# facebookresearch/esm

Measured on NVIDIA H100. Metric: sequences/sec ESM-2 650M L=1024 embedding extract, higher is better.
Workload: dtype f16 operands, f32 accumulate/residual/LayerNorm/softmax

## Files before the change

### esm_b200/csrc/api.cu

```cuda
#include "../../include/esmb200.h"

#include <cuda.h>
#include <cuda_runtime.h>
#include <stdio.h>
#include <stdlib.h>
#include <string.h>

#include <string>
#include <vector>

#include <mutex>

#include "attention8.cuh"
#include "attention_contact.cuh"
#include "attention_probs.cuh"
#include "common.cuh"
#include "elementwise.cuh"
#include "gemm2.cuh"
#include "gemm_fp8.cuh"
#include "jacobian.cuh"
#include "msa_select.cuh"
#include "sampling.cuh"
#include "tied_attention.cuh"

using namespace esmb200;

namespace {

thread_local std::string g_last_error;

int fail(int code, const std::string& msg) {
  g_last_error = msg;
  return code;
}

int fail_cuda(cudaError_t e, const char* what) {
  if (e == cudaErrorMemoryAllocation)
    return fail(ESMB200_ENOMEM, std::string("CUDA out of memory. (") + what + ")");
  return fail(ESMB200_ECUDA, std::string(what) + ": " + cudaGetErrorString(e));
}

#define CK(expr)                                        \
  do {                                                  \
    cudaError_t _e = (expr);                            \
    if (_e != cudaSuccess) return fail_cuda(_e, #expr); \
  } while (0)


enum ProfTag : int { T_LN1 = 0, T_QKV, T_ATTN, T_OUT, T_LN2, T_FC1, T_FC2, T_KEYBITS, T_EMBED, T_LN_F32, T_PROBS,
                     T_CONVERT, T_GEMM_OTHER, T_MEANPOOL, T_TIED_SCORES, T_TIED_SOFTMAX, T_TIED_PV, T_LOG_SOFTMAX,
                     T_WINDOW_MERGE, T_JACOBIAN, T_SAMPLING, T_MSA_SELECT, T_COUNT };
struct Profiler {
  std::mutex mu;
  bool on = false;
  std::vector<cudaEvent_t> ev;
  std::vector<int> tag;
  size_t used = 0;
  long long launches = 0;
};
Profiler g_prof;

struct ProfScope {
  cudaStream_t st;
  bool rec;
  size_t slot = 0;
  ProfScope(int tag, cudaStream_t s) : st(s), rec(false) {
    std::lock_guard<std::mutex> lk(g_prof.mu);
    ++g_prof.launches;
    if (g_prof.on && g_prof.used + 2 <= g_prof.ev.size()) {
      rec = true;
      slot = g_prof.used;
      g_prof.used += 2;
      g_prof.tag.push_back(tag);
      cudaEventRecord(g_prof.ev[slot], st);
    }
  }
  ~ProfScope() {
    if (rec) cudaEventRecord(g_prof.ev[slot + 1], st);
  }
};

typedef CUresult (*EncodeTiledFn)(CUtensorMap*, CUtensorMapDataType, cuuint32_t, void*, const cuuint64_t*,
                                  const cuuint64_t*, const cuuint32_t*, const cuuint32_t*, CUtensorMapInterleave,
                                  CUtensorMapSwizzle, CUtensorMapL2promotion, CUtensorMapFloatOOBfill);

EncodeTiledFn get_encode_fn() {
  static EncodeTiledFn fn = nullptr;
  if (fn) return fn;
  void* p = nullptr;
  cudaDriverEntryPointQueryResult qres;
  if (cudaGetDriverEntryPoint("cuTensorMapEncodeTiled", &p, cudaEnableDefault, &qres) != cudaSuccess ||
      qres != cudaDriverEntryPointSuccess)
    return nullptr;
  fn = reinterpret_cast<EncodeTiledFn>(p);
  return fn;
}

int make_tmap_2d(CUtensorMap* map, const void* ptr, int esize, uint64_t rows, uint64_t cols, uint64_t ld_elems,
                 uint32_t box_rows) {
  EncodeTiledFn enc = get_encode_fn();
  if (!enc) return fail(ESMB200_ECUDA, "cuTensorMapEncodeTiled entry point not available");
  if ((reinterpret_cast<uintptr_t>(ptr) & 15) != 0 || (ld_elems * esize) % 16 != 0)
    return fail(ESMB200_EINVAL, "TMA operand must be 16-byte aligned with a 16-byte multiple row pitch");
  cuuint64_t dims[2] = {cols, rows};
  cuuint64_t strides[1] = {ld_elems * (uint64_t)esize};
  cuuint32_t box[2] = {(cuuint32_t)(128 / esize), box_rows};
  cuuint32_t estr[2] = {1, 1};
  const CUtensorMapDataType dt = esize == 1   ? CU_TENSOR_MAP_DATA_TYPE_UINT8
                                 : esize == 2 ? CU_TENSOR_MAP_DATA_TYPE_FLOAT16
                                              : CU_TENSOR_MAP_DATA_TYPE_FLOAT32;
  CUresult r = enc(map, dt, 2,
                   const_cast<void*>(ptr), dims, strides, box, estr,
                   CU_TENSOR_MAP_INTERLEAVE_NONE, CU_TENSOR_MAP_SWIZZLE_128B, CU_TENSOR_MAP_L2_PROMOTION_L2_256B,
                   CU_TENSOR_MAP_FLOAT_OOB_FILL_NONE);
  if (r != CUDA_SUCCESS) {
    char buf[160];
    snprintf(buf, sizeof buf, "cuTensorMapEncodeTiled failed (%d) rows=%llu cols=%llu ld=%llu box_rows=%u", (int)r,
             (unsigned long long)rows, (unsigned long long)cols, (unsigned long long)ld_elems, box_rows);
    return fail(ESMB200_ECUDA, buf);
  }
  return ESMB200_OK;
}

int make_tmap_f16(CUtensorMap* map, const void* ptr, uint64_t rows, uint64_t cols, uint64_t ld_elems,
                  uint32_t box_rows) {
  return make_tmap_2d(map, ptr, 2, rows, cols, ld_elems, box_rows);
}

int make_gemm_out_map(CUtensorMap* map, const void* out, int esize, uint64_t rows, uint64_t cols) {
  return make_tmap_2d(map, out, esize, rows, cols, cols, gemm2_cfg::OUT_BOX_ROWS);
}

inline int head_slots(int E, int H) { return (H > 0 && E / H > 64) ? 2 : 1; }

constexpr int kMaxDevices = 64;

int num_sms() {
  static int n[kMaxDevices] = {};
  int dev = 0;
  cudaGetDevice(&dev);
  if (dev < 0 || dev >= kMaxDevices) dev = 0;
  if (n[dev] == 0) cudaDeviceGetAttribute(&n[dev], cudaDevAttrMultiProcessorCount, dev);
  return n[dev];
}

int check_device() {
  static int ok[kMaxDevices] = {};
  int dev = 0;
  if (cudaGetDevice(&dev) != cudaSuccess) return fail(ESMB200_ECUDA, "no CUDA device");
  if (dev < 0 || dev >= kMaxDevices) return fail(ESMB200_ECUDA, "device ordinal out of range");
  if (ok[dev] == 0) {
    int major = 0;
    cudaDeviceGetAttribute(&major, cudaDevAttrComputeCapabilityMajor, dev);
    ok[dev] = (major == 9) ? 1 : -1;
  }
  if (ok[dev] < 0)
    return fail(ESMB200_ECUDA, "esmb200 requires an sm_90a (Hopper H100) device; there is no fallback path");
  return ESMB200_OK;
}

size_t align_up(size_t v, size_t a) { return (v + a - 1) / a * a; }

constexpr int kContactMaxS = 1024;
const char* const kContactMaxSMsg = "contact head supports at most 1024 positions";

template <bool SPLIT>
cudaError_t launch_gemm_epi(int epi, const CUtensorMap& ta, const CUtensorMap& tb, const CUtensorMap& to,
                            const GemmParams& p, cudaStream_t st) {
  switch (epi) {
    case EPI_QKV_ROPE: return launch_gemm2_epi<EPI_QKV_ROPE, SPLIT>(ta, tb, to, p, num_sms(), st);
    case EPI_BIAS_RESIDUAL: return launch_gemm2_epi<EPI_BIAS_RESIDUAL, SPLIT>(ta, tb, to, p, num_sms(), st);
    case EPI_BIAS_GELU: return launch_gemm2_epi<EPI_BIAS_GELU, SPLIT>(ta, tb, to, p, num_sms(), st);
    case EPI_BIAS_F32: return launch_gemm2_epi<EPI_BIAS_F32, SPLIT>(ta, tb, to, p, num_sms(), st);
    case EPI_BIAS_GELU_F32: return launch_gemm2_epi<EPI_BIAS_GELU_F32, SPLIT>(ta, tb, to, p, num_sms(), st);
    default: return cudaErrorInvalidValue;
  }
}

int launch_gemm(int epi, const CUtensorMap& ta, const CUtensorMap& tb, const CUtensorMap& to, const GemmParams& p,
                cudaStream_t st, int tag = T_GEMM_OTHER, bool split = false) {
  ProfScope ps(tag, st);
  if (split && p.K % 64 != 0) return fail(ESMB200_EINVAL, "fp32x3 precision needs K % 64 == 0");
  if (epi < EPI_QKV_ROPE || epi > EPI_BIAS_GELU_F32) return fail(ESMB200_EINVAL, "unknown GEMM epilogue");
  const cudaError_t e =
      split ? launch_gemm_epi<true>(epi, ta, tb, to, p, st) : launch_gemm_epi<false>(epi, ta, tb, to, p, st);
  if (e != cudaSuccess) return fail_cuda(e, split ? "gemm launch (fp32x3)" : "gemm launch");
  return ESMB200_OK;
}

int launch_gemm_fp8(int epi, const CUtensorMap& ta, const CUtensorMap& tb, const CUtensorMap& to, const Fp8GemmParams& p,
                    cudaStream_t st, int tag = T_GEMM_OTHER) {
  ProfScope ps(tag, st);
  cudaError_t e;
  switch (epi) {
    case EPI_QKV_ROPE: e = launch_gemm_fp8_epi<EPI_QKV_ROPE>(ta, tb, to, p, num_sms(), st); break;
    case EPI_BIAS_RESIDUAL: e = launch_gemm_fp8_epi<EPI_BIAS_RESIDUAL>(ta, tb, to, p, num_sms(), st); break;
    case EPI_GELU_FP8: e = launch_gemm_fp8_epi<EPI_GELU_FP8>(ta, tb, to, p, num_sms(), st); break;
    default: return fail(ESMB200_EINVAL, "fp8 gemm epilogue must be 0 (qkv), 1 (residual) or 5 (gelu -> fp8)");
  }
  if (e != cudaSuccess) return fail_cuda(e, "gemm launch (fp8)");
  return ESMB200_OK;
}

inline int kblocks(int K) { return (K + 127) / 128; }

GemmParams gemm_params(int M, int N, int K, const float* bias) {
  GemmParams g;
  memset(&g, 0, sizeof g);
  g.M = M; g.N = N; g.K = K; g.bias = bias;
  return g;
}

struct AttnScratch {
  uint32_t* keybits;
  int* kvlen;
  float* row_max;
  float* row_sum;
  int words;
  size_t bytes;
};

AttnScratch attn_scratch_layout(uintptr_t base, int B, int T, int H) {
  AttnScratch s;
  s.words = (int)align_up((size_t)(T + 31) / 32, 4);
  const size_t keybits = align_up((size_t)B * s.words * 4, 256), kvlen = align_up((size_t)B * 4, 256);
  const size_t stats = align_up((size_t)B * H * T * 4, 256);
  s.keybits = reinterpret_cast<uint32_t*>(base);
  s.kvlen = reinterpret_cast<int*>(base + keybits);
  s.row_max = reinterpret_cast<float*>(base + keybits + kvlen);
  s.row_sum = reinterpret_cast<float*>(base + keybits + kvlen + stats);
  s.bytes = keybits + kvlen + 2 * stats;
  return s;
}

int run_key_bits(const uint8_t* pad_mask, const AttnScratch& s, int B, int T, cudaStream_t st) {
  const int wpb = 4;
  ProfScope ps(T_KEYBITS, st);
  key_bits_kernel<<<(B + wpb - 1) / wpb, wpb * 32, 0, st>>>(pad_mask, s.keybits, s.kvlen, B, T, s.words);
  CK(cudaGetLastError());
  return ESMB200_OK;
}

struct ContactLayer {
  const float* w;
  const uint8_t* keep;
  float* acc;
  float* row_part;
  float* col_part;
  int lo, S;
};

int run_probs(const CUtensorMap& tq, ProbsParams pp, cudaStream_t st, const char* what) {
  const int per = probs_cfg::seqs_per_launch(pp.H);
  for (int b0 = 0; b0 < pp.B; b0 += per) {
    pp.b0 = b0;
    cudaError_t e;
    {
      ProfScope ps(T_PROBS, st);
      e = launch_attention_probs(tq, pp, pp.B - b0 < per ? pp.B - b0 : per, st);
    }
    if (e != cudaSuccess) return fail_cuda(e, what);
  }
  return ESMB200_OK;
}

int run_attention(const void* qkv, void* ctx, float* probs, long long probs_batch_stride, int attn_flags,
                  const AttnScratch& s, int B, int T, int H, cudaStream_t st, bool split = false,
                  const ContactLayer* contact = nullptr, int slots = 1) {
  const int E = H * 64 * slots;
  if (slots == 2 && split) return fail(ESMB200_EINVAL, "head_dim > 64: fp32x3 precision is not available");
  const uint64_t qcols = (uint64_t)(split ? 6 : 3) * E;
  CUtensorMap tq;
  int rc = make_tmap_f16(&tq, qkv, (uint64_t)B * T, qcols, qcols, 128);
  if (rc) return rc;
  AttnParams ap;
  ap.B = B; ap.T = T; ap.H = H; ap.E = E;
  ap.lo_off = split ? 3 * E : 0;
  ap.slots = slots;
  ap.keybits = s.keybits; ap.kvlen = s.kvlen; ap.words = s.words;
  ap.ctx = static_cast<__half*>(ctx);
  ap.row_max = probs || contact ? s.row_max : nullptr;
  ap.row_sum = probs || contact ? s.row_sum : nullptr;
  cudaError_t e;
  {
    CUtensorMap tkv;
    rc = make_tmap_f16(&tkv, qkv, (uint64_t)B * T, qcols, qcols, attention_fwd_kv_box_rows(ap));
    if (rc) return rc;
    ProfScope ps(T_ATTN, st);
    e = launch_attention_fwd(tq, tkv, ap, num_sms(), st);
  }
  if (e != cudaSuccess) return fail_cuda(e, "attention launch");
  if (contact && !split) {
    if (B > 65535) return fail(ESMB200_EINVAL, "return_contacts: B must be <= 65535");
    ContactFuseParams cp;
    cp.B = B; cp.T = T; cp.H = H; cp.E = E; cp.slots = slots;
    cp.keybits = s.keybits; cp.kvlen = s.kvlen; cp.words = s.words;
    cp.row_max = s.row_max; cp.row_sum = s.row_sum; cp.probs = probs;
    cp.batch_stride = probs_batch_stride > 0 ? probs_batch_stride : (long long)H * T * T;
    cp.zero_pad_rows = attn_flags & 1;
    cp.w = contact->w; cp.keep = contact->keep; cp.acc = contact->acc;
    cp.row_part = contact->row_part; cp.col_part = contact->col_part; cp.lo = contact->lo; cp.S = contact->S;
    {
      ProfScope ps(T_PROBS, st);
      e = launch_attention_probs_contact(tq, cp, st);
    }
    if (e != cudaSuccess) return fail_cuda(e, "attention probs+contact launch");
    return ESMB200_OK;
  }
  if (probs) {
    ProbsParams pp;
    pp.B = B; pp.T = T; pp.H = H; pp.E = E;
    pp.keybits = s.keybits; pp.kvlen = s.kvlen; pp.words = s.words;
    pp.row_max = s.row_max; pp.row_sum = s.row_sum; pp.probs = probs;
    pp.batch_stride = probs_batch_stride > 0 ? probs_batch_stride : (long long)H * T * T;
    pp.zero_pad_rows = attn_flags & 1;
    pp.lo_off = split ? 3 * E : 0;
    pp.slots = slots;
    return run_probs(tq, pp, st, "attention probs launch");
  }
  return ESMB200_OK;
}

int run_contact_accumulate(const float* attn, long long batch_stride, const float* w, const uint8_t* keep, float* acc,
                           float* row_sum, float* col_part, int B, int H, int T, int lo, int S, cudaStream_t st) {
  ProfScope ps(T_PROBS, st);
  const size_t smem = (size_t)8 * S * sizeof(float);
  dim3 grid((S + 15) / 16, B);
  if (S <= 512)
    contact_accumulate_kernel<2, 16, 2><<<grid, 256, smem, st>>>(attn, batch_stride, w, keep, acc, row_sum, col_part, H, T,
                                                                  lo, S);
  else
    contact_accumulate_kernel<2, 32, 1><<<grid, 256, smem, st>>>(attn, batch_stride, w, keep, acc, row_sum, col_part, H, T,
                                                                  lo, S);
  CK(cudaGetLastError());
  return ESMB200_OK;
}

int run_column_attention(const void* qkv, void* ctx, const AttnScratch& s, int B, int R, int C, int H,
                         cudaStream_t st, bool split = false, float* probs = nullptr) {
  const int E = H * 64;
  AttnParams ap;
  ap.B = B * C; ap.T = R; ap.H = H; ap.E = E;
  ap.lo_off = split ? 3 * E : 0;
  ap.keybits = s.keybits; ap.kvlen = s.kvlen; ap.words = s.words;
  ap.ctx = static_cast<__half*>(ctx);
  ap.row_max = probs ? s.row_max : nullptr;
  ap.row_sum = probs ? s.row_sum : nullptr;
  ap.cols = C;
  CUtensorMap tq, tkv;
  const uint64_t wide = (uint64_t)C * (split ? 6 : 3) * E;
  int rc;
  if ((rc = make_tmap_f16(&tq, qkv, (uint64_t)B * R, wide, wide, 128))) return rc;
  if ((rc = make_tmap_f16(&tkv, qkv, (uint64_t)B * R, wide, wide, attention_fwd_kv_box_rows(ap)))) return rc;
  cudaError_t e;
  {
    ProfScope ps(T_ATTN, st);
    e = launch_attention_fwd(tq, tkv, ap, num_sms(), st);
  }
  if (e != cudaSuccess) return fail_cuda(e, "column attention launch");
  if (probs) {
    ProbsParams pp;
    pp.B = B * C; pp.T = R; pp.H = H; pp.E = E;
    pp.keybits = s.keybits; pp.kvlen = s.kvlen; pp.words = s.words;
    pp.row_max = s.row_max; pp.row_sum = s.row_sum; pp.probs = probs;
    pp.batch_stride = (long long)H * R * R;
    pp.zero_pad_rows = 0;
    pp.lo_off = ap.lo_off;
    pp.cols = C;
    return run_probs(tq, pp, st, "column attention probs launch");
  }
  return ESMB200_OK;
}

int layernorm_f16(const float* x, const float* w, const float* b, void* out, int M, int E, float eps, bool split,
                  int tag, cudaStream_t st) {
  cudaError_t e;
  {
    ProfScope ps(tag, st);
    e = split ? launch_layernorm<2>(x, w, b, out, M, E, eps, st) : launch_layernorm<1>(x, w, b, out, M, E, eps, st);
  }
  if (e != cudaSuccess) return fail_cuda(e, split ? "layernorm_split" : "layernorm_f16");
  return ESMB200_OK;
}

int layernorm_fp8(const float* x, const float* w, const float* b, void* out, float* scales, int M, int E, float eps,
                  int tag, cudaStream_t st) {
  cudaError_t e;
  {
    ProfScope ps(tag, st);
    e = launch_layernorm<3>(x, w, b, out, M, E, eps, st, scales);
  }
  if (e != cudaSuccess) return fail_cuda(e, "layernorm_fp8");
  return ESMB200_OK;
}

int quantize_fp8(const float* src, uint8_t* dst, float* scales, int rows, int K, int block_rows, cudaStream_t st) {
  ProfScope ps(T_CONVERT, st);
  quantize_fp8_kernel<<<dim3(kblocks(K), (rows + block_rows - 1) / block_rows), 256, 0, st>>>(src, dst, scales, rows, K,
                                                                                               block_rows);
  CK(cudaGetLastError());
  return ESMB200_OK;
}

int convert_f16(const float* src, void* dst, size_t rows, int K, bool split, cudaStream_t st) {
  const size_t n = rows * (size_t)K;
  size_t blocks = (n + 255) / 256;
  if (blocks > (size_t)num_sms() * 16) blocks = (size_t)num_sms() * 16;
  ProfScope ps(T_CONVERT, st);
  if (split)
    convert_f32_split_kernel<<<(unsigned)blocks, 256, 0, st>>>(src, static_cast<__half*>(dst), rows, K);
  else
    convert_f32_f16_kernel<<<(unsigned)blocks, 256, 0, st>>>(src, static_cast<__half*>(dst), n);
  CK(cudaGetLastError());
  return ESMB200_OK;
}

}

struct WeightMaps {
  CUtensorMap qkv, out, fc1, fc2;
};

struct esmb200_layer {
  int E, H, F;
  int d;
  int slots;
  int Ea;
  float q_scale;
  int split;
  int fp8;
  float eps;
  const float *ln1_w, *ln1_b, *ln2_w, *ln2_b, *out_b, *fc1_b, *fc2_b;
  __half* w_qkv;
  __half* w_out;
  __half* w_fc1;
  __half* w_fc2;
  float* b_qkv;
  uint8_t* w8;
  uint8_t *q_qkv, *q_fc1, *q_fc2;
  float *s_qkv, *s_fc1, *s_fc2;
  WeightMaps tm;
  const void* host;
};

namespace {
struct PackedLayout {
  size_t qkv, out, fc1, fc2;
  size_t bytes;
};

PackedLayout packed_layout(int E, int H, int F, int split) {
  const size_t pf = split ? 2 : 1, Ea = (size_t)64 * head_slots(E, H) * H;
  PackedLayout p;
  p.qkv = 0;
  p.out = align_up(3 * Ea * E * 2 * pf, 1024);
  p.fc1 = p.out + align_up(Ea * E * 2 * pf, 1024);
  p.fc2 = p.fc1 + align_up((size_t)F * E * 2 * pf, 1024);
  p.bytes = p.fc2 + align_up((size_t)E * F * 2 * pf, 1024);
  return p;
}

struct Fp8Layout {
  size_t qkv, fc1, fc2, s_qkv, s_fc1, s_fc2;
  size_t bytes;
};

Fp8Layout fp8_layout(int E, int Ea, int F) {
  Fp8Layout l;
  size_t o = 0;
  auto take = [&](size_t n) {
    const size_t at = o;
    o += align_up(n, 1024);
    return at;
  };
  l.qkv = take((size_t)3 * Ea * E);
  l.fc1 = take((size_t)F * E);
  l.fc2 = take((size_t)E * F);
// ... 1224 lines not shown
```

### esm_b200/csrc/common.cuh

```cuda
#pragma once

#include <cuda.h>
#include <cuda_fp16.h>
#include <cuda_runtime.h>
#include <stdint.h>
#include <stdio.h>
#include <stdlib.h>

#ifndef ESMB200_WATCHDOG
#define ESMB200_WATCHDOG 1
#endif

namespace esmb200 {

constexpr uint32_t kWarp = 32;

__device__ __forceinline__ uint32_t smem_u32(const void* p) {
  return static_cast<uint32_t>(__cvta_generic_to_shared(p));
}

__device__ __forceinline__ uint32_t lane_id() {
  uint32_t r;
  asm volatile("mov.u32 %0, %%laneid;" : "=r"(r));
  return r;
}

__device__ __forceinline__ bool elect_one() {
  uint32_t pred = 0;
  asm volatile(
      "{\n\t"
      ".reg .pred P1;\n\t"
      "elect.sync _|P1, 0xffffffff;\n\t"
      "selp.u32 %0, 1, 0, P1;\n\t"
      "}\n"
      : "=r"(pred));
  return pred != 0;
}

__device__ __forceinline__ void mbar_init(uint64_t* bar, uint32_t count) {
  asm volatile("mbarrier.init.shared::cta.b64 [%0], %1;" ::"r"(smem_u32(bar)), "r"(count) : "memory");
}

__device__ __forceinline__ void fence_barrier_init() {
  asm volatile("fence.mbarrier_init.release.cluster;" ::: "memory");
}

__device__ __forceinline__ void fence_proxy_async_smem() {
  asm volatile("fence.proxy.async.shared::cta;" ::: "memory");
}

__device__ __forceinline__ void mbar_arrive(uint64_t* bar) {
  asm volatile("mbarrier.arrive.shared::cta.b64 _, [%0];" ::"r"(smem_u32(bar)) : "memory");
}

__device__ __forceinline__ void mbar_arrive_expect_tx(uint64_t* bar, uint32_t bytes) {
  asm volatile("mbarrier.arrive.expect_tx.shared::cta.b64 _, [%0], %1;" ::"r"(smem_u32(bar)), "r"(bytes)
               : "memory");
}

__device__ __forceinline__ bool mbar_try_wait(uint64_t* bar, uint32_t parity) {
  uint32_t ok;
  asm volatile(
      "{\n\t"
      ".reg .pred p;\n\t"
      "mbarrier.try_wait.parity.shared::cta.b64 p, [%1], %2;\n\t"
      "selp.u32 %0, 1, 0, p;\n\t"
      "}\n"
      : "=r"(ok)
      : "r"(smem_u32(bar)), "r"(parity)
      : "memory");
  return ok != 0;
}

__device__ __forceinline__ void mbar_wait(uint64_t* bar, uint32_t parity) {
  if (mbar_try_wait(bar, parity)) return;
#if ESMB200_WATCHDOG
  uint32_t polls = 0;
  while (!mbar_try_wait(bar, parity)) {
    if (++polls == (1u << 26)) {
      printf("esmb200: mbarrier watchdog block=(%d,%d,%d) thread=%d bar=%u parity=%u\n", blockIdx.x, blockIdx.y,
             blockIdx.z, threadIdx.x, smem_u32(bar), parity);
      __trap();
    }
  }
#else
  while (!mbar_try_wait(bar, parity)) {
  }
#endif
}


__device__ __forceinline__ void mbar_wait_relaxed(uint64_t* bar, uint32_t parity) {
  if (mbar_try_wait(bar, parity)) return;
#if ESMB200_WATCHDOG
  uint32_t polls = 0;
#endif
  while (!mbar_try_wait(bar, parity)) {
    __nanosleep(200);
#if ESMB200_WATCHDOG
    if (++polls == (1u << 24)) {
      printf("esmb200: mbarrier watchdog (relaxed) block=(%d,%d,%d) thread=%d bar=%u parity=%u\n", blockIdx.x, blockIdx.y,
             blockIdx.z, threadIdx.x, smem_u32(bar), parity);
      __trap();
    }
#endif
  }
}

__device__ __forceinline__ void tma_prefetch_desc(const CUtensorMap* map) {
  asm volatile("prefetch.tensormap [%0];" ::"l"(reinterpret_cast<uint64_t>(map)) : "memory");
}

__device__ __forceinline__ void tma_load_2d(void* smem_dst, const CUtensorMap* map, uint64_t* bar, int32_t c0,
                                            int32_t c1) {
  asm volatile(
      "cp.async.bulk.tensor.2d.shared::cluster.global.mbarrier::complete_tx::bytes [%0], [%1, {%3, %4}], [%2];"
      :
      : "r"(smem_u32(smem_dst)), "l"(reinterpret_cast<uint64_t>(map)), "r"(smem_u32(bar)), "r"(c0), "r"(c1)
      : "memory");
}

__device__ __forceinline__ void tma_load_2d_addr(uint32_t smem_dst, const CUtensorMap* map, uint32_t bar, int32_t c0,
                                                 int32_t c1) {
  asm volatile(
      "cp.async.bulk.tensor.2d.shared::cluster.global.mbarrier::complete_tx::bytes [%0], [%1, {%3, %4}], [%2];"
      :
      : "r"(smem_dst), "l"(reinterpret_cast<uint64_t>(map)), "r"(bar), "r"(c0), "r"(c1)
      : "memory");
}
__device__ __forceinline__ void mbar_arrive_expect_tx_addr(uint32_t bar, uint32_t bytes) {
  asm volatile("mbarrier.arrive.expect_tx.shared::cta.b64 _, [%0], %1;" ::"r"(bar), "r"(bytes) : "memory");
}

__device__ __forceinline__ void tma_load_2d_hint(void* smem_dst, const CUtensorMap* map, uint64_t* bar, int32_t c0,
                                                 int32_t c1, uint64_t policy) {
  asm volatile(
      "cp.async.bulk.tensor.2d.shared::cluster.global.mbarrier::complete_tx::bytes.L2::cache_hint [%0], [%1, {%3, "
      "%4}], [%2], %5;"
      :
      : "r"(smem_u32(smem_dst)), "l"(reinterpret_cast<uint64_t>(map)), "r"(smem_u32(bar)), "r"(c0), "r"(c1),
        "l"(policy)
      : "memory");
}

__device__ __forceinline__ uint64_t l2_policy_evict_last() {
  uint64_t p;
  asm volatile("createpolicy.fractional.L2::evict_last.b64 %0, 1.0;" : "=l"(p));
  return p;
}
__device__ __forceinline__ uint64_t l2_policy_evict_first() {
  uint64_t p;
  asm volatile("createpolicy.fractional.L2::evict_first.b64 %0, 1.0;" : "=l"(p));
  return p;
}

__device__ __forceinline__ void mma16816(float (&d)[4], const uint32_t (&a)[4], uint32_t b0, uint32_t b1) {
  asm volatile(
      "mma.sync.aligned.m16n8k16.row.col.f32.f16.f16.f32 {%0, %1, %2, %3}, {%4, %5, %6, %7}, {%8, %9}, "
      "{%0, %1, %2, %3};"
      : "+f"(d[0]), "+f"(d[1]), "+f"(d[2]), "+f"(d[3])
      : "r"(a[0]), "r"(a[1]), "r"(a[2]), "r"(a[3]), "r"(b0), "r"(b1));
}

__device__ __forceinline__ void ldsm_x4(uint32_t addr, uint32_t (&r)[4]) {
  asm volatile("ldmatrix.sync.aligned.m8n8.x4.shared.b16 {%0, %1, %2, %3}, [%4];"
               : "=r"(r[0]), "=r"(r[1]), "=r"(r[2]), "=r"(r[3])
               : "r"(addr));
}
__device__ __forceinline__ void ldsm_x4_t(uint32_t addr, uint32_t (&r)[4]) {
  asm volatile("ldmatrix.sync.aligned.m8n8.x4.trans.shared.b16 {%0, %1, %2, %3}, [%4];"
               : "=r"(r[0]), "=r"(r[1]), "=r"(r[2]), "=r"(r[3])
               : "r"(addr));
}

__device__ __forceinline__ void stsm_x4(uint32_t addr, uint32_t r0, uint32_t r1, uint32_t r2, uint32_t r3) {
  asm volatile("stmatrix.sync.aligned.m8n8.x4.shared.b16 [%0], {%1, %2, %3, %4};" ::"r"(addr), "r"(r0), "r"(r1),
               "r"(r2), "r"(r3)
               : "memory");
}
__device__ __forceinline__ void st_shared_f32x2(uint32_t addr, float a, float b) {
  asm volatile("st.shared.v2.f32 [%0], {%1, %2};" ::"r"(addr), "f"(a), "f"(b) : "memory");
}

__device__ __forceinline__ uint32_t sw128(uint32_t base, uint32_t row, uint32_t chunk) {
  return base + row * 128u + ((chunk ^ (row & 7u)) << 4);
}

__device__ __forceinline__ void ldsm_a(uint32_t base, uint32_t r0, uint32_t kk, uint32_t (&a)[4]) {
  const uint32_t l = lane_id();
  ldsm_x4(sw128(base, r0 + (l & 15u), 2u * kk + (l >> 4)), a);
}
__device__ __forceinline__ void ldsm_b(uint32_t base, uint32_t n0, uint32_t kk, uint32_t (&b)[4]) {
  const uint32_t l = lane_id();
  ldsm_x4(sw128(base, n0 + (l & 7u) + ((l >> 4) << 3), 2u * kk + ((l >> 3) & 1u)), b);
}
__device__ __forceinline__ void ldsm_bt(uint32_t base, uint32_t kk, uint32_t n0, uint32_t (&b)[4]) {
  const uint32_t l = lane_id();
  ldsm_x4_t(sw128(base, 16u * kk + (l & 15u), n0 / 8u + (l >> 4)), b);
}

__device__ __forceinline__ uint64_t wgmma_desc_sw128(uint32_t smem_addr) {
  uint64_t d = 0;
  d |= static_cast<uint64_t>((smem_addr & 0x3FFFFu) >> 4);
  d |= static_cast<uint64_t>(1) << 16;
  d |= static_cast<uint64_t>(1024 >> 4) << 32;
  d |= static_cast<uint64_t>(1) << 62;
  return d;
}

__device__ __forceinline__ void wgmma_fence() { asm volatile("wgmma.fence.sync.aligned;" ::: "memory"); }
__device__ __forceinline__ void wgmma_commit() { asm volatile("wgmma.commit_group.sync.aligned;" ::: "memory"); }
template <int N>
__device__ __forceinline__ void wgmma_wait() {
  asm volatile("wgmma.wait_group.sync.aligned %0;" ::"n"(N) : "memory");
}
template <int N>
__device__ __forceinline__ void reg_fence_f(float (&r)[N]) {
#pragma unroll
  for (int i = 0; i < N; ++i) asm volatile("" : "+f"(r[i])::"memory");
}

__device__ __forceinline__ void wgmma_m64n256k16(float (&d)[128], uint64_t da, uint64_t db, int scale_d) {
  asm volatile(
      "{\n.reg .pred p;\nsetp.ne.b32 p, %130, 0;\n"
      "wgmma.mma_async.sync.aligned.m64n256k16.f32.f16.f16 "
      "{%0, %1, %2, %3, %4, %5, %6, %7, %8, %9, %10, %11, %12, %13, %14, %15, "
      "%16, %17, %18, %19, %20, %21, %22, %23, %24, %25, %26, %27, %28, %29, %30, %31, "
      "%32, %33, %34, %35, %36, %37, %38, %39, %40, %41, %42, %43, %44, %45, %46, %47, "
      "%48, %49, %50, %51, %52, %53, %54, %55, %56, %57, %58, %59, %60, %61, %62, %63, "
      "%64, %65, %66, %67, %68, %69, %70, %71, %72, %73, %74, %75, %76, %77, %78, %79, "
      "%80, %81, %82, %83, %84, %85, %86, %87, %88, %89, %90, %91, %92, %93, %94, %95, "
      "%96, %97, %98, %99, %100, %101, %102, %103, %104, %105, %106, %107, %108, %109, %110, %111, "
      "%112, %113, %114, %115, %116, %117, %118, %119, %120, %121, %122, %123, %124, %125, %126, %127}, "
      "%128, %129, p, 1, 1, 0, 0;\n}\n"
      : "+f"(d[0]), "+f"(d[1]), "+f"(d[2]), "+f"(d[3]), "+f"(d[4]), "+f"(d[5]), "+f"(d[6]), "+f"(d[7]),
        "+f"(d[8]), "+f"(d[9]), "+f"(d[10]), "+f"(d[11]), "+f"(d[12]), "+f"(d[13]), "+f"(d[14]), "+f"(d[15]),
        "+f"(d[16]), "+f"(d[17]), "+f"(d[18]), "+f"(d[19]), "+f"(d[20]), "+f"(d[21]), "+f"(d[22]), "+f"(d[23]),
        "+f"(d[24]), "+f"(d[25]), "+f"(d[26]), "+f"(d[27]), "+f"(d[28]), "+f"(d[29]), "+f"(d[30]), "+f"(d[31]),
        "+f"(d[32]), "+f"(d[33]), "+f"(d[34]), "+f"(d[35]), "+f"(d[36]), "+f"(d[37]), "+f"(d[38]), "+f"(d[39]),
        "+f"(d[40]), "+f"(d[41]), "+f"(d[42]), "+f"(d[43]), "+f"(d[44]), "+f"(d[45]), "+f"(d[46]), "+f"(d[47]),
        "+f"(d[48]), "+f"(d[49]), "+f"(d[50]), "+f"(d[51]), "+f"(d[52]), "+f"(d[53]), "+f"(d[54]), "+f"(d[55]),
        "+f"(d[56]), "+f"(d[57]), "+f"(d[58]), "+f"(d[59]), "+f"(d[60]), "+f"(d[61]), "+f"(d[62]), "+f"(d[63]),
        "+f"(d[64]), "+f"(d[65]), "+f"(d[66]), "+f"(d[67]), "+f"(d[68]), "+f"(d[69]), "+f"(d[70]), "+f"(d[71]),
        "+f"(d[72]), "+f"(d[73]), "+f"(d[74]), "+f"(d[75]), "+f"(d[76]), "+f"(d[77]), "+f"(d[78]), "+f"(d[79]),
        "+f"(d[80]), "+f"(d[81]), "+f"(d[82]), "+f"(d[83]), "+f"(d[84]), "+f"(d[85]), "+f"(d[86]), "+f"(d[87]),
        "+f"(d[88]), "+f"(d[89]), "+f"(d[90]), "+f"(d[91]), "+f"(d[92]), "+f"(d[93]), "+f"(d[94]), "+f"(d[95]),
        "+f"(d[96]), "+f"(d[97]), "+f"(d[98]), "+f"(d[99]), "+f"(d[100]), "+f"(d[101]), "+f"(d[102]), "+f"(d[103]),
        "+f"(d[104]), "+f"(d[105]), "+f"(d[106]), "+f"(d[107]), "+f"(d[108]), "+f"(d[109]), "+f"(d[110]), "+f"(d[111]),
        "+f"(d[112]), "+f"(d[113]), "+f"(d[114]), "+f"(d[115]), "+f"(d[116]), "+f"(d[117]), "+f"(d[118]), "+f"(d[119]),
        "+f"(d[120]), "+f"(d[121]), "+f"(d[122]), "+f"(d[123]), "+f"(d[124]), "+f"(d[125]), "+f"(d[126]), "+f"(d[127])
      : "l"(da), "l"(db), "r"(scale_d));
}

__device__ __forceinline__ uint64_t wgmma_desc_sw128_mn(uint32_t smem_addr) {
  uint64_t d = 0;
  d |= static_cast<uint64_t>((smem_addr & 0x3FFFFu) >> 4);
  d |= static_cast<uint64_t>(1024 >> 4) << 16;
  d |= static_cast<uint64_t>(1024 >> 4) << 32;
  d |= static_cast<uint64_t>(1) << 62;
  return d;
}

__device__ __forceinline__ void wgmma_m64n128k16(float (&d)[64], uint64_t da, uint64_t db, int scale_d) {
  asm volatile(
      "{\n.reg .pred p;\nsetp.ne.b32 p, %66, 0;\n"
      "wgmma.mma_async.sync.aligned.m64n128k16.f32.f16.f16 "
      "{%0, %1, %2, %3, %4, %5, %6, %7, %8, %9, %10, %11, %12, %13, %14, %15, "
      "%16, %17, %18, %19, %20, %21, %22, %23, %24, %25, %26, %27, %28, %29, %30, %31, "
      "%32, %33, %34, %35, %36, %37, %38, %39, %40, %41, %42, %43, %44, %45, %46, %47, "
      "%48, %49, %50, %51, %52, %53, %54, %55, %56, %57, %58, %59, %60, %61, %62, %63}, "
      "%64, %65, p, 1, 1, 0, 0;\n}\n"
      : "+f"(d[0]), "+f"(d[1]), "+f"(d[2]), "+f"(d[3]), "+f"(d[4]), "+f"(d[5]), "+f"(d[6]), "+f"(d[7]),
        "+f"(d[8]), "+f"(d[9]), "+f"(d[10]), "+f"(d[11]), "+f"(d[12]), "+f"(d[13]), "+f"(d[14]), "+f"(d[15]),
        "+f"(d[16]), "+f"(d[17]), "+f"(d[18]), "+f"(d[19]), "+f"(d[20]), "+f"(d[21]), "+f"(d[22]), "+f"(d[23]),
        "+f"(d[24]), "+f"(d[25]), "+f"(d[26]), "+f"(d[27]), "+f"(d[28]), "+f"(d[29]), "+f"(d[30]), "+f"(d[31]),
        "+f"(d[32]), "+f"(d[33]), "+f"(d[34]), "+f"(d[35]), "+f"(d[36]), "+f"(d[37]), "+f"(d[38]), "+f"(d[39]),
        "+f"(d[40]), "+f"(d[41]), "+f"(d[42]), "+f"(d[43]), "+f"(d[44]), "+f"(d[45]), "+f"(d[46]), "+f"(d[47]),
        "+f"(d[48]), "+f"(d[49]), "+f"(d[50]), "+f"(d[51]), "+f"(d[52]), "+f"(d[53]), "+f"(d[54]), "+f"(d[55]),
        "+f"(d[56]), "+f"(d[57]), "+f"(d[58]), "+f"(d[59]), "+f"(d[60]), "+f"(d[61]), "+f"(d[62]), "+f"(d[63])
      : "l"(da), "l"(db), "r"(scale_d));
}

__device__ __forceinline__ void wgmma_m64n64k16_rs(float (&d)[32], const uint32_t (&a)[4], uint64_t db) {
  asm volatile(
      "{\n.reg .pred p;\nsetp.ne.b32 p, 1, 0;\n"
      "wgmma.mma_async.sync.aligned.m64n64k16.f32.f16.f16 "
      "{%0, %1, %2, %3, %4, %5, %6, %7, %8, %9, %10, %11, %12, %13, %14, %15, "
      "%16, %17, %18, %19, %20, %21, %22, %23, %24, %25, %26, %27, %28, %29, %30, %31}, "
      "{%32, %33, %34, %35}, %36, p, 1, 1, 1;\n}\n"
      : "+f"(d[0]), "+f"(d[1]), "+f"(d[2]), "+f"(d[3]), "+f"(d[4]), "+f"(d[5]), "+f"(d[6]), "+f"(d[7]),
        "+f"(d[8]), "+f"(d[9]), "+f"(d[10]), "+f"(d[11]), "+f"(d[12]), "+f"(d[13]), "+f"(d[14]), "+f"(d[15]),
        "+f"(d[16]), "+f"(d[17]), "+f"(d[18]), "+f"(d[19]), "+f"(d[20]), "+f"(d[21]), "+f"(d[22]), "+f"(d[23]),
        "+f"(d[24]), "+f"(d[25]), "+f"(d[26]), "+f"(d[27]), "+f"(d[28]), "+f"(d[29]), "+f"(d[30]), "+f"(d[31])
      : "r"(a[0]), "r"(a[1]), "r"(a[2]), "r"(a[3]), "l"(db));
}

template <uint32_t R>
__device__ __forceinline__ void setmaxnreg_dec() { asm volatile("setmaxnreg.dec.sync.aligned.u32 %0;" ::"n"(R)); }
template <uint32_t R>
__device__ __forceinline__ void setmaxnreg_inc() { asm volatile("setmaxnreg.inc.sync.aligned.u32 %0;" ::"n"(R)); }

__device__ __forceinline__ void tma_store_2d(const CUtensorMap* map, const void* smem_src, int32_t c0, int32_t c1) {
  asm volatile("cp.async.bulk.tensor.2d.global.shared::cta.bulk_group [%0, {%2, %3}], [%1];" ::"l"(
                   reinterpret_cast<uint64_t>(map)),
               "r"(smem_u32(smem_src)), "r"(c0), "r"(c1)
               : "memory");
}
__device__ __forceinline__ void tma_reduce_add_2d(const CUtensorMap* map, const void* smem_src, int32_t c0,
                                                  int32_t c1) {
  asm volatile("cp.reduce.async.bulk.tensor.2d.global.shared::cta.add.tile.bulk_group [%0, {%2, %3}], [%1];" ::"l"(
                   reinterpret_cast<uint64_t>(map)),
               "r"(smem_u32(smem_src)), "r"(c0), "r"(c1)
               : "memory");
}
__device__ __forceinline__ void tma_store_commit() { asm volatile("cp.async.bulk.commit_group;" ::: "memory"); }
template <int N>
__device__ __forceinline__ void tma_store_wait_read() {
  asm volatile("cp.async.bulk.wait_group.read %0;" ::"n"(N) : "memory");
}
__device__ __forceinline__ void tma_store_wait_all() { asm volatile("cp.async.bulk.wait_group 0;" ::: "memory"); }

__device__ __forceinline__ void pdl_wait() { asm volatile("griddepcontrol.wait;" ::: "memory"); }
__device__ __forceinline__ void pdl_launch_dependents() { asm volatile("griddepcontrol.launch_dependents;" ::: "memory"); }

inline int& pdl_flag() {
  static int flag = -1;
  return flag;
}
inline bool pdl_enabled() {
  int& f = pdl_flag();
  if (f < 0) {
    const char* e = getenv("ESMB200_PDL");
    f = (e && e[0] == '1') ? 1 : 0;
  }
  return f != 0;
}

template <typename... KArgs, typename... Args>
inline cudaError_t launch_pdl(void (*kernel)(KArgs...), dim3 grid, dim3 block, size_t smem, cudaStream_t stream,
                              Args&&... args) {
  cudaLaunchConfig_t cfg = {};
  cfg.gridDim = grid;
  cfg.blockDim = block;
  cfg.dynamicSmemBytes = smem;
  cfg.stream = stream;
  cudaLaunchAttribute attr[1];
  attr[0].id = cudaLaunchAttributeProgrammaticStreamSerialization;
  attr[0].val.programmaticStreamSerializationAllowed = 1;
  cfg.attrs = attr;
  cfg.numAttrs = pdl_enabled() ? 1 : 0;
  return cudaLaunchKernelEx(&cfg, kernel, KArgs(args)...);
}

__device__ __forceinline__ uint32_t pack_half2(float lo, float hi) {
  __half2 h = __floats2half2_rn(lo, hi);
  return *reinterpret_cast<uint32_t*>(&h);
}

__device__ __forceinline__ void fma2(float& d0, float& d1, float a0, float a1, float b0, float b1, float c0, float c1) {
  d0 = fmaf(a0, b0, c0);
  d1 = fmaf(a1, b1, c1);
}
__device__ __forceinline__ void add2(float& d0, float& d1, float a0, float a1, float b0, float b1) {
  d0 = a0 + b0;
  d1 = a1 + b1;
}
__device__ __forceinline__ void mul2(float& d0, float& d1, float a0, float a1, float b0, float b1) {
  d0 = a0 * b0;
  d1 = a1 * b1;
}

__device__ __forceinline__ float ex2_approx(float x) {
  float y;
  asm("ex2.approx.ftz.f32 %0, %1;" : "=f"(y) : "f"(x));
  return y;
}

__device__ __forceinline__ float warp_sum(float v) {
#pragma unroll
  for (int o = 16; o > 0; o >>= 1) v += __shfl_xor_sync(0xffffffffu, v, o);
  return v;
}

__device__ __forceinline__ float fp8_block_scale(float amax) {
  if (amax == 0.f) return 1.0f;
  const uint32_t b = __float_as_uint(amax);
  const int e = (int)(b >> 23) - 8 + ((b & 0x7fffffu) > 0x600000u ? 1 : 0);
  return __uint_as_float((uint32_t)(e < 1 ? 1 : e) << 23);
}
__device__ __forceinline__ uint16_t cvt_e4m3x2(float lo, float hi) {
  uint16_t r;
  asm("cvt.rn.satfinite.e4m3x2.f32 %0, %1, %2;" : "=h"(r) : "f"(hi), "f"(lo));
  return r;
}
__device__ __forceinline__ float warp_max(float v) {
#pragma unroll
  for (int o = 16; o > 0; o >>= 1) v = fmaxf(v, __shfl_xor_sync(0xffffffffu, v, o));
  return v;
}

__device__ __forceinline__ void named_bar_sync(uint32_t id, uint32_t nthreads) {
  asm volatile("bar.sync %0, %1;" ::"r"(id), "r"(nthreads) : "memory");
}
__device__ __forceinline__ void named_bar_arrive(uint32_t id, uint32_t nthreads) {
  asm volatile("bar.arrive %0, %1;" ::"r"(id), "r"(nthreads) : "memory");
}

}
```

### esm_b200/csrc/gemm2.cuh

```cuda
#pragma once

#include "gemm_common.cuh"

namespace esmb200 {

namespace gemm2_cfg {
constexpr int BLOCK_M = 128;
constexpr int BLOCK_N = 256;
constexpr int HALF_N = 128;
constexpr int BLOCK_K = 64;
constexpr int STAGES = 4;
constexpr int A_STAGE_BYTES = BLOCK_M * BLOCK_K * 2;
constexpr int B_STAGE_BYTES = BLOCK_N * BLOCK_K * 2;
constexpr int STAGE_BYTES = A_STAGE_BYTES + B_STAGE_BYTES;
constexpr int BOX_M = 128;
constexpr int OUT_BOX_ROWS = 64;
constexpr int OUT_BOX_BYTES = OUT_BOX_ROWS * 128;
constexpr int OUT_BUFS = 2;
constexpr int NUM_THREADS = 384;
constexpr int SMEM_BYTES = STAGES * STAGE_BYTES + 2 * OUT_BUFS * OUT_BOX_BYTES + 1024 + 256;
}

template <int EPI, bool SPLIT = false>
__global__ void __launch_bounds__(gemm2_cfg::NUM_THREADS, 1)
gemm2_f16_kernel(const __grid_constant__ CUtensorMap tmap_a, const __grid_constant__ CUtensorMap tmap_b,
                 const __grid_constant__ CUtensorMap tmap_o, const GemmParams p) {
  using namespace gemm2_cfg;
  extern __shared__ uint8_t smem_raw[];
  uint8_t* smem = reinterpret_cast<uint8_t*>((reinterpret_cast<uintptr_t>(smem_raw) + 1023) & ~uintptr_t(1023));
  uint8_t* smem_a = smem;
  uint8_t* smem_b = smem + STAGES * A_STAGE_BYTES;
  uint8_t* smem_out = smem + STAGES * STAGE_BYTES;
  uint64_t* bars = reinterpret_cast<uint64_t*>(smem_out + 2 * OUT_BUFS * OUT_BOX_BYTES);
  uint64_t* full_bar = bars;
  uint64_t* empty_bar = bars + STAGES;

  const uint32_t wg = __shfl_sync(0xffffffffu, threadIdx.x / 128, 0);
  const int tiles_m = (p.M + BLOCK_M - 1) / BLOCK_M;
  const int tiles_n = (p.N + BLOCK_N - 1) / BLOCK_N;
  const int num_tiles = tiles_m * tiles_n;
  const int num_kb1 = (p.K + BLOCK_K - 1) / BLOCK_K;
  const int num_kb = SPLIT ? 3 * num_kb1 : num_kb1;

  if (threadIdx.x == 0) {
    tma_prefetch_desc(&tmap_a);
    tma_prefetch_desc(&tmap_b);
    tma_prefetch_desc(&tmap_o);
    for (int i = 0; i < STAGES; ++i) {
      mbar_init(&full_bar[i], 1);
      mbar_init(&empty_bar[i], 2);
    }
    fence_barrier_init();
  }
  __syncthreads();
  pdl_launch_dependents();
  pdl_wait();

  if (wg == 0) {
    setmaxnreg_dec<40>();
    if (threadIdx.x == 0) {
      uint32_t it = 0;
      for (int tile = blockIdx.x; tile < num_tiles; tile += gridDim.x) {
        const int m0 = (tile / tiles_n) * BLOCK_M, n0 = (tile % tiles_n) * BLOCK_N;
        for (int kb = 0; kb < num_kb; ++kb, ++it) {
          const uint32_t s = it % STAGES;
          while (!mbar_try_wait(&empty_bar[s], ((it / STAGES) & 1) ^ 1)) __nanosleep(64);
          int a_col = kb * BLOCK_K, b_col = kb * BLOCK_K;
          if constexpr (SPLIT) {
            const int part = kb % 3;
            a_col = (kb / 3) * BLOCK_K + (part == 1 ? p.K : 0);
            b_col = (kb / 3) * BLOCK_K + (part == 2 ? p.K : 0);
          }
          mbar_arrive_expect_tx(&full_bar[s], STAGE_BYTES);
          tma_load_2d(smem_a + s * A_STAGE_BYTES, &tmap_a, &full_bar[s], a_col, m0);
          tma_load_2d(smem_b + s * B_STAGE_BYTES, &tmap_b, &full_bar[s], b_col, n0);
          tma_load_2d(smem_b + s * B_STAGE_BYTES + HALF_N * 128, &tmap_b, &full_bar[s], b_col, n0 + HALF_N);
        }
      }
    }
    return;
  }

  setmaxnreg_inc<232>();
  const uint32_t mw = wg - 1;
  const uint32_t warp = (threadIdx.x / 32) % 4;
  const uint32_t lane = threadIdx.x % 32;
  const uint32_t g = lane / 4, c = lane % 4;
  const bool signal = (threadIdx.x % 128) == 0;
  const uint32_t a_base = smem_u32(smem_a) + mw * 64 * 128;
  const uint32_t b_base = smem_u32(smem_b);
  uint8_t* const out_bufs = smem_out + mw * OUT_BUFS * OUT_BOX_BYTES;
  uint32_t ob = 0;
  uint32_t it = 0;
  float acc[128];

  auto store_box = [&](int c0, int c1) {
    fence_proxy_async_smem();
    if (signal) tma_store_wait_read<0>();
    named_bar_sync(1 + mw, 128);
    if (signal) {
      if constexpr (EPI == EPI_BIAS_RESIDUAL) {
        tma_reduce_add_2d(&tmap_o, out_bufs + ob * OUT_BOX_BYTES, c0, c1);
      } else {
        tma_store_2d(&tmap_o, out_bufs + ob * OUT_BOX_BYTES, c0, c1);
      }
      tma_store_commit();
    }
    ob ^= 1;
  };

  for (int tile = blockIdx.x; tile < num_tiles; tile += gridDim.x) {
    const int m0 = (tile / tiles_n) * BLOCK_M, n0 = (tile % tiles_n) * BLOCK_N;
    for (int kb = 0; kb < num_kb; ++kb, ++it) {
      const uint32_t s = it % STAGES;
      while (!mbar_try_wait(&full_bar[s], (it / STAGES) & 1)) {
      }
      wgmma_fence();
      const uint64_t da = wgmma_desc_sw128(a_base + s * A_STAGE_BYTES);
      const uint64_t db = wgmma_desc_sw128(b_base + s * B_STAGE_BYTES);
#pragma unroll
      for (int k = 0; k < BLOCK_K / 16; ++k) wgmma_m64n256k16(acc, da + 2 * k, db + 2 * k, (kb | k) != 0);
      wgmma_commit();
      wgmma_wait<1>();
      if (kb > 0 && signal) mbar_arrive(&empty_bar[(it + STAGES - 1) % STAGES]);
    }
    wgmma_wait<0>();
    reg_fence_f(acc);
    if (signal) mbar_arrive(&empty_bar[(it + STAGES - 1) % STAGES]);

    const int r0 = m0 + (int)(mw * 64 + warp * 16 + g);
    const int box_row = m0 + (int)mw * 64;
    if constexpr (EPI == EPI_QKV_ROPE || EPI == EPI_BIAS_GELU) {
#pragma unroll
      for (int gi = 0; gi < 4; ++gi) {
        const int col0 = n0 + gi * 64;
        if (col0 >= p.N) break;
        uint32_t hi[16], lo[16];
        if constexpr (EPI == EPI_QKV_ROPE) {
          epi_qkv_box<SPLIT>(acc + 32 * gi, p, col0, r0, c, hi, lo);
        } else {
#pragma unroll
          for (int b = 0; b < 8; ++b) {
            const int i = 8 * gi + b;
            const float2 bb = __ldg(reinterpret_cast<const float2*>(p.bias + col0 + 8 * b + 2 * (int)c));
#pragma unroll
            for (int hr = 0; hr < 2; ++hr) {
              const float y0 = gelu_erf(acc[4 * i + 2 * hr] + bb.x), y1 = gelu_erf(acc[4 * i + 2 * hr + 1] + bb.y);
              hi[2 * b + hr] = pack_half2(y0, y1);
              if constexpr (SPLIT) {
                const float2 f = __half22float2(*reinterpret_cast<const __half2*>(&hi[2 * b + hr]));
                lo[2 * b + hr] = pack_half2(y0 - f.x, y1 - f.y);
              }
            }
          }
        }
        stage_box_f16(smem_u32(out_bufs + ob * OUT_BOX_BYTES), warp, lane, hi);
        store_box(col0, box_row);
        if constexpr (SPLIT) {
          stage_box_f16(smem_u32(out_bufs + ob * OUT_BOX_BYTES), warp, lane, lo);
          store_box(p.lo_col_off + col0, box_row);
        }
      }
    } else {
#pragma unroll
      for (int gi = 0; gi < 8; ++gi) {
        const int col0 = n0 + gi * 32;
        if (col0 >= p.N) break;
        const uint32_t buf = smem_u32(out_bufs + ob * OUT_BOX_BYTES);
#pragma unroll
        for (int b = 0; b < 4; ++b) {
          const int i = 4 * gi + b;
          const float2 bb = col0 + 8 * b < p.N
                                ? __ldg(reinterpret_cast<const float2*>(p.bias + col0 + 8 * b + 2 * (int)c))
                                : make_float2(0.f, 0.f);
#pragma unroll
          for (int hr = 0; hr < 2; ++hr) {
            float y0 = acc[4 * i + 2 * hr] + bb.x, y1 = acc[4 * i + 2 * hr + 1] + bb.y;
            if constexpr (EPI == EPI_BIAS_GELU_F32) {
              y0 = gelu_erf(y0);
              y1 = gelu_erf(y1);
            }
            st_shared_f32x2(sw128(buf, warp * 16 + 8 * hr + g, 2 * b + c / 2) + (c % 2) * 8, y0, y1);
          }
        }
        store_box(col0, box_row);
      }
    }
  }
  if (signal) tma_store_wait_all();
}

template <int EPI, bool SPLIT = false>
inline cudaError_t launch_gemm2_epi(const CUtensorMap& ta, const CUtensorMap& tb, const CUtensorMap& to,
                                    const GemmParams& p, int num_sms, cudaStream_t stream) {
  using namespace gemm2_cfg;
  cudaError_t e =
      cudaFuncSetAttribute(gemm2_f16_kernel<EPI, SPLIT>, cudaFuncAttributeMaxDynamicSharedMemorySize, SMEM_BYTES);
  if (e != cudaSuccess) return e;
  const int tiles = ((p.M + BLOCK_M - 1) / BLOCK_M) * ((p.N + BLOCK_N - 1) / BLOCK_N);
  const int grid = tiles < num_sms ? tiles : num_sms;
  return launch_pdl(gemm2_f16_kernel<EPI, SPLIT>, dim3(grid), dim3(NUM_THREADS), SMEM_BYTES, stream, ta, tb, to, p);
}

}
```

Measured before the change: 321.2.

## Use 2-CTA clusters with TMA multicast of B tiles in persistent GEMM

The persistent GEMM now launches as 2-CTA clusters. The two CTAs work on vertically adjacent M tiles that share the same N tile, and each CTA loads half of the B tile and multicasts it to both. Each empty barrier now waits for four arrivals, from both consumers in both CTAs, and cluster syncs are added at startup and teardown. The aim is to halve L2-to-SM traffic for the weight operand. In exchange the two CTAs run in lockstep, cluster scheduling can reduce the number of resident CTAs, and odd tile_m counts may leave a partner doing out-of-range work.

```diff
diff --git a/esm_b200/csrc/api.cu b/esm_b200/csrc/api.cu
--- a/esm_b200/csrc/api.cu
+++ b/esm_b200/csrc/api.cu
@@ -168,11 +168,11 @@
 cudaError_t launch_gemm_epi(int epi, const CUtensorMap& ta, const CUtensorMap& tb, const CUtensorMap& to,
                             const GemmParams& p, cudaStream_t st) {
   switch (epi) {
-    case EPI_QKV_ROPE: return launch_gemm2_epi<EPI_QKV_ROPE, SPLIT>(ta, tb, to, p, num_sms(), st);
-    case EPI_BIAS_RESIDUAL: return launch_gemm2_epi<EPI_BIAS_RESIDUAL, SPLIT>(ta, tb, to, p, num_sms(), st);
-    case EPI_BIAS_GELU: return launch_gemm2_epi<EPI_BIAS_GELU, SPLIT>(ta, tb, to, p, num_sms(), st);
-    case EPI_BIAS_F32: return launch_gemm2_epi<EPI_BIAS_F32, SPLIT>(ta, tb, to, p, num_sms(), st);
-    case EPI_BIAS_GELU_F32: return launch_gemm2_epi<EPI_BIAS_GELU_F32, SPLIT>(ta, tb, to, p, num_sms(), st);
+    case EPI_QKV_ROPE: return launch_gemm2_epi<EPI_QKV_ROPE, SPLIT>(ta, tb, to, p, st);
+    case EPI_BIAS_RESIDUAL: return launch_gemm2_epi<EPI_BIAS_RESIDUAL, SPLIT>(ta, tb, to, p, st);
+    case EPI_BIAS_GELU: return launch_gemm2_epi<EPI_BIAS_GELU, SPLIT>(ta, tb, to, p, st);
+    case EPI_BIAS_F32: return launch_gemm2_epi<EPI_BIAS_F32, SPLIT>(ta, tb, to, p, st);
+    case EPI_BIAS_GELU_F32: return launch_gemm2_epi<EPI_BIAS_GELU_F32, SPLIT>(ta, tb, to, p, st);
     default: return cudaErrorInvalidValue;
   }
 }
diff --git a/esm_b200/csrc/common.cuh b/esm_b200/csrc/common.cuh
--- a/esm_b200/csrc/common.cuh
+++ b/esm_b200/csrc/common.cuh
@@ -51,6 +51,17 @@
 
 __device__ __forceinline__ void mbar_arrive(uint64_t* bar) {
   asm volatile("mbarrier.arrive.shared::cta.b64 _, [%0];" ::"r"(smem_u32(bar)) : "memory");
+}
+
+__device__ __forceinline__ void mbar_arrive_cluster(uint64_t* bar, uint32_t cta) {
+  asm volatile(
+      "{\n\t"
+      ".reg .b32 ra;\n\t"
+      "mapa.shared::cluster.u32 ra, %0, %1;\n\t"
+      "mbarrier.arrive.shared::cluster.b64 _, [ra];\n\t"
+      "}\n" ::"r"(smem_u32(bar)),
+      "r"(cta)
+      : "memory");
 }
 
 __device__ __forceinline__ void mbar_arrive_expect_tx(uint64_t* bar, uint32_t bytes) {
@@ -117,6 +128,17 @@
       "cp.async.bulk.tensor.2d.shared::cluster.global.mbarrier::complete_tx::bytes [%0], [%1, {%3, %4}], [%2];"
       :
       : "r"(smem_u32(smem_dst)), "l"(reinterpret_cast<uint64_t>(map)), "r"(smem_u32(bar)), "r"(c0), "r"(c1)
+      : "memory");
+}
+
+__device__ __forceinline__ void tma_load_2d_multicast(void* smem_dst, const CUtensorMap* map, uint64_t* bar, int32_t c0,
+                                                      int32_t c1, uint16_t cta_mask) {
+  asm volatile(
+      "cp.async.bulk.tensor.2d.shared::cluster.global.mbarrier::complete_tx::bytes.multicast::cluster"
+      " [%0], [%1, {%3, %4}], [%2], %5;"
+      :
+      : "r"(smem_u32(smem_dst)), "l"(reinterpret_cast<uint64_t>(map)), "r"(smem_u32(bar)), "r"(c0), "r"(c1),
+        "h"(cta_mask)
       : "memory");
 }
 
@@ -337,19 +359,35 @@
 }
 
 template <typename... KArgs, typename... Args>
-inline cudaError_t launch_pdl(void (*kernel)(KArgs...), dim3 grid, dim3 block, size_t smem, cudaStream_t stream,
-                              Args&&... args) {
+inline cudaError_t launch_pdl_cluster(int cluster, void (*kernel)(KArgs...), dim3 grid, dim3 block, size_t smem,
+                                      cudaStream_t stream, Args&&... args) {
   cudaLaunchConfig_t cfg = {};
   cfg.gridDim = grid;
   cfg.blockDim = block;
   cfg.dynamicSmemBytes = smem;
   cfg.stream = stream;
-  cudaLaunchAttribute attr[1];
-  attr[0].id = cudaLaunchAttributeProgrammaticStreamSerialization;
-  attr[0].val.programmaticStreamSerializationAllowed = 1;
+  cudaLaunchAttribute attr[2];
+  int n = 0;
+  if (cluster > 1) {
+    attr[n].id = cudaLaunchAttributeClusterDimension;
+    attr[n].val.clusterDim.x = (unsigned)cluster;
+    attr[n].val.clusterDim.y = 1;
+    attr[n].val.clusterDim.z = 1;
+    ++n;
+  }
+  if (pdl_enabled()) {
+    attr[n].id = cudaLaunchAttributeProgrammaticStreamSerialization;
+    attr[n].val.programmaticStreamSerializationAllowed = 1;
+    ++n;
+  }
   cfg.attrs = attr;
-  cfg.numAttrs = pdl_enabled() ? 1 : 0;
+  cfg.numAttrs = n;
   return cudaLaunchKernelEx(&cfg, kernel, KArgs(args)...);
+}
+template <typename... KArgs, typename... Args>
+inline cudaError_t launch_pdl(void (*kernel)(KArgs...), dim3 grid, dim3 block, size_t smem, cudaStream_t stream,
+                              Args&&... args) {
+  return launch_pdl_cluster(1, kernel, grid, block, smem, stream, static_cast<Args&&>(args)...);
 }
 
 __device__ __forceinline__ uint32_t pack_half2(float lo, float hi) {
@@ -406,4 +444,13 @@
   asm volatile("bar.arrive %0, %1;" ::"r"(id), "r"(nthreads) : "memory");
 }
 
-}
+__device__ __forceinline__ uint32_t cluster_ctarank() {
+  uint32_t r;
+  asm volatile("mov.u32 %0, %%cluster_ctarank;" : "=r"(r));
+  return r;
+}
+__device__ __forceinline__ void cluster_sync() {
+  asm volatile("barrier.cluster.arrive.release;\n\tbarrier.cluster.wait.acquire;" ::: "memory");
+}
+
+}
diff --git a/esm_b200/csrc/gemm2.cuh b/esm_b200/csrc/gemm2.cuh
--- a/esm_b200/csrc/gemm2.cuh
+++ b/esm_b200/csrc/gemm2.cuh
@@ -36,9 +36,11 @@
   uint64_t* empty_bar = bars + STAGES;
 
   const uint32_t wg = __shfl_sync(0xffffffffu, threadIdx.x / 128, 0);
+  const uint32_t rank = cluster_ctarank();
   const int tiles_m = (p.M + BLOCK_M - 1) / BLOCK_M;
   const int tiles_n = (p.N + BLOCK_N - 1) / BLOCK_N;
-  const int num_tiles = tiles_m * tiles_n;
+  const int num_pairs = (tiles_m + 1) / 2 * tiles_n;
+  const int cluster = blockIdx.x / 2, num_clusters = gridDim.x / 2;
   const int num_kb1 = (p.K + BLOCK_K - 1) / BLOCK_K;
   const int num_kb = SPLIT ? 3 * num_kb1 : num_kb1;
 
@@ -48,11 +50,11 @@
     tma_prefetch_desc(&tmap_o);
     for (int i = 0; i < STAGES; ++i) {
       mbar_init(&full_bar[i], 1);
-      mbar_init(&empty_bar[i], 2);
+      mbar_init(&empty_bar[i], 4);
     }
     fence_barrier_init();
   }
-  __syncthreads();
+  cluster_sync();
   pdl_launch_dependents();
   pdl_wait();
 
@@ -60,8 +62,8 @@
     setmaxnreg_dec<40>();
     if (threadIdx.x == 0) {
       uint32_t it = 0;
-      for (int tile = blockIdx.x; tile < num_tiles; tile += gridDim.x) {
-        const int m0 = (tile / tiles_n) * BLOCK_M, n0 = (tile % tiles_n) * BLOCK_N;
+      for (int pair = cluster; pair < num_pairs; pair += num_clusters) {
+        const int m0 = (2 * (pair / tiles_n) + (int)rank) * BLOCK_M, n0 = (pair % tiles_n) * BLOCK_N;
         for (int kb = 0; kb < num_kb; ++kb, ++it) {
           const uint32_t s = it % STAGES;
           while (!mbar_try_wait(&empty_bar[s], ((it / STAGES) & 1) ^ 1)) __nanosleep(64);
@@ -73,11 +75,12 @@
           }
           mbar_arrive_expect_tx(&full_bar[s], STAGE_BYTES);
           tma_load_2d(smem_a + s * A_STAGE_BYTES, &tmap_a, &full_bar[s], a_col, m0);
-          tma_load_2d(smem_b + s * B_STAGE_BYTES, &tmap_b, &full_bar[s], b_col, n0);
-          tma_load_2d(smem_b + s * B_STAGE_BYTES + HALF_N * 128, &tmap_b, &full_bar[s], b_col, n0 + HALF_N);
-        }
-      }
-    }
+          tma_load_2d_multicast(smem_b + s * B_STAGE_BYTES + rank * (HALF_N * 128), &tmap_b, &full_bar[s], b_col,
+                                n0 + (int)rank * HALF_N, 0x3);
+        }
+      }
+    }
+    cluster_sync();
     return;
   }
 
@@ -109,8 +112,13 @@
     ob ^= 1;
   };
 
-  for (int tile = blockIdx.x; tile < num_tiles; tile += gridDim.x) {
-    const int m0 = (tile / tiles_n) * BLOCK_M, n0 = (tile % tiles_n) * BLOCK_N;
+  auto release = [&](uint32_t s) {
+    mbar_arrive(&empty_bar[s]);
+    mbar_arrive_cluster(&empty_bar[s], rank ^ 1);
+  };
+
+  for (int pair = cluster; pair < num_pairs; pair += num_clusters) {
+    const int m0 = (2 * (pair / tiles_n) + (int)rank) * BLOCK_M, n0 = (pair % tiles_n) * BLOCK_N;
     for (int kb = 0; kb < num_kb; ++kb, ++it) {
       const uint32_t s = it % STAGES;
       while (!mbar_try_wait(&full_bar[s], (it / STAGES) & 1)) {
@@ -122,11 +130,11 @@
       for (int k = 0; k < BLOCK_K / 16; ++k) wgmma_m64n256k16(acc, da + 2 * k, db + 2 * k, (kb | k) != 0);
       wgmma_commit();
       wgmma_wait<1>();
-      if (kb > 0 && signal) mbar_arrive(&empty_bar[(it + STAGES - 1) % STAGES]);
+      if (kb > 0 && signal) release((it + STAGES - 1) % STAGES);
     }
     wgmma_wait<0>();
     reg_fence_f(acc);
-    if (signal) mbar_arrive(&empty_bar[(it + STAGES - 1) % STAGES]);
+    if (signal) release((it + STAGES - 1) % STAGES);
 
     const int r0 = m0 + (int)(mw * 64 + warp * 16 + g);
     const int box_row = m0 + (int)mw * 64;
@@ -188,18 +196,52 @@
     }
   }
   if (signal) tma_store_wait_all();
+  cluster_sync();
+}
+
+template <int EPI, bool SPLIT>
+inline cudaError_t gemm2_max_clusters(int* clusters) {
+  using namespace gemm2_cfg;
+  static int n[64] = {};
+  int dev = 0;
+  cudaGetDevice(&dev);
+  if (dev < 0 || dev >= 64) dev = 0;
+  if (n[dev] == 0) {
+    cudaLaunchConfig_t cfg = {};
+    cfg.gridDim = dim3(2);
+    cfg.blockDim = dim3(NUM_THREADS);
+    cfg.dynamicSmemBytes = SMEM_BYTES;
+    cudaLaunchAttribute attr[1];
+    attr[0].id = cudaLaunchAttributeClusterDimension;
+    attr[0].val.clusterDim.x = 2;
+    attr[0].val.clusterDim.y = 1;
+    attr[0].val.clusterDim.z = 1;
+    cfg.attrs = attr;
+    cfg.numAttrs = 1;
+    int c = 0;
+    const cudaError_t e = cudaOccupancyMaxActiveClusters(&c, gemm2_f16_kernel<EPI, SPLIT>, &cfg);
+    if (e != cudaSuccess) return e;
+    if (c <= 0) return cudaErrorInvalidConfiguration;
+    n[dev] = c;
+  }
+  *clusters = n[dev];
+  return cudaSuccess;
 }
 
 template <int EPI, bool SPLIT = false>
 inline cudaError_t launch_gemm2_epi(const CUtensorMap& ta, const CUtensorMap& tb, const CUtensorMap& to,
-                                    const GemmParams& p, int num_sms, cudaStream_t stream) {
+                                    const GemmParams& p, cudaStream_t stream) {
   using namespace gemm2_cfg;
   cudaError_t e =
       cudaFuncSetAttribute(gemm2_f16_kernel<EPI, SPLIT>, cudaFuncAttributeMaxDynamicSharedMemorySize, SMEM_BYTES);
   if (e != cudaSuccess) return e;
-  const int tiles = ((p.M + BLOCK_M - 1) / BLOCK_M) * ((p.N + BLOCK_N - 1) / BLOCK_N);
-  const int grid = tiles < num_sms ? tiles : num_sms;
-  return launch_pdl(gemm2_f16_kernel<EPI, SPLIT>, dim3(grid), dim3(NUM_THREADS), SMEM_BYTES, stream, ta, tb, to, p);
-}
-
-}
+  int clusters = 0;
+  e = gemm2_max_clusters<EPI, SPLIT>(&clusters);
+  if (e != cudaSuccess) return e;
+  const int pairs = ((p.M + BLOCK_M - 1) / BLOCK_M + 1) / 2 * ((p.N + BLOCK_N - 1) / BLOCK_N);
+  const int grid = 2 * (pairs < clusters ? pairs : clusters);
+  return launch_pdl_cluster(2, gemm2_f16_kernel<EPI, SPLIT>, dim3(grid), dim3(NUM_THREADS), SMEM_BYTES, stream, ta,
+                            tb, to, p);
+}
+
+}
```

Result: faster. 326.7, median of 6 (+1.7%).
